# wzn0828/Adaptive

Hardware: AMD Instinct MI355X
Metric: captions/sec (greedy, max_len=20) at B=512; 1/2/4/8-GPU scaling (higher is better)
Workload: dtype fp32; 1 GPU; greedy decode (Encoder2Decoder.sampler) B=512/GPU, max_len=20; batch_per_gpu=512, global_batch=512, max_len=20, hidden=512, embed=256, vocab=10123, parallelism=dp1, batches_in_flight=1, feature_buffers=3, headline=one sampler() call after another on resident batches

## Files before the change

### adaptive_amd/csrc/aa_encoder.hip

```cpp
#include "aa_internal.hpp"

namespace aa {

__global__ __launch_bounds__(256) void k_avgpool(const float* __restrict__ feats, int64_t nch, float* __restrict__ a_g) {
  __shared__ float buf[4][64 * P];
  const int lane = threadIdx.x & 63, w = threadIdx.x >> 6;
  const int64_t ch0 = ((int64_t)blockIdx.x * 4 + w) * 64;
  const int nhere = ch0 < nch ? (int)(nch - ch0 < 64 ? nch - ch0 : 64) : 0;
  const int nf4 = nhere * P / 4;
  const float4* src = reinterpret_cast<const float4*>(feats + ch0 * P);
  float4* dst = reinterpret_cast<float4*>(buf[w]);
  for (int q = lane; q < nf4; q += 64) dst[q] = src[q];
  __syncthreads();
  if (lane < nhere) {
    const float* row = buf[w] + lane * P;
    float s = 0.f;
    for (int p = 0; p < P; ++p) s += row[p];
    a_g[ch0 + lane] = s / 49.0f;
  }
}

template <int BM>
struct ANCHW {
  const float* base;
  __device__ __forceinline__ void init(const float* F, int C, int m0, int M) {
    const int m = m0 + (int)(threadIdx.x % BM);
    const int mc = m < M ? m : M - 1;
    const int b = mc / P, p = mc - b * P;
    base = F + (int64_t)b * C * P + p;
  }
  __device__ __forceinline__ void map(int q, int& r, int& kq) const { r = q % BM; kq = q / BM; }
  __device__ __forceinline__ float4 load(int , int q, int k0) const {
    const float* s = base + (k0 + 4 * (q / BM)) * P;
    return make_float4(s[0], s[P], s[2 * P], s[3 * P]);
  }
};

__global__ __launch_bounds__(256) void k_enc_v(const float* __restrict__ feats, int B, int C, int H,
                                               const float* __restrict__ W, const float* __restrict__ bias,
                                               float* __restrict__ V) {
  constexpr int BM = 64, BN = 64;
  __shared__ __attribute__((aligned(16))) float lds[Tile<BM, BN>::LDS_FLOATS];
  const int M = B * P, MT = (M + BM - 1) / BM, NTn = H / BN;
  const int L = xcd_remap(blockIdx.x, MT * NTn);
  const int mt = L / NTn, nt = L % NTn;
  ANCHW<BM> al;
  al.init(feats, C, mt * BM, M);
  WRowMajor wl{W, C, nt * BN};
  floatx16 acc[1][1];
  gemm_mainloop<BM, BN>(al, wl, C / BK, lds, acc);
  const int lane = threadIdx.x & 63, wave = threadIdx.x >> 6, wm = wave >> 1, wn = wave & 1;
  const int col = nt * BN + wn * 32 + (lane & 31);
  const float bv = bias[col];
#pragma unroll
  for (int r = 0; r < 16; ++r) {
    const int row = mt * BM + wm * 32 + acc_row(r, lane);
    if (row < M) V[(int64_t)row * H + col] = reluf_(acc[0][0][r] + bv);
  }
}

constexpr int EV_BM = 128, EV_BN = 128, EV_BK = 32, EV_LD = 40;


__global__ __launch_bounds__(256, 2) void k_enc_v3(const float* __restrict__ feats, int B, int C, int H,
                                                   const bf16x8* __restrict__ W3, const float* __restrict__ bias,
                                                   float* __restrict__ V) {
  __shared__ __attribute__((aligned(16))) __bf16 As[2][3][EV_BM * EV_LD];
  const int M = B * P, MT = (M + EV_BM - 1) / EV_BM, NTn = H / EV_BN, KC = C / 16;
  const int L = xcd_remap(blockIdx.x, MT * NTn);
  const int mt = L / NTn, nt = L % NTn;
  const int t = threadIdx.x, lane = t & 63, wave = t >> 6;
  const int li = lane & 31, lh = lane >> 5;
  const int r = t & (EV_BM - 1), kh = t >> 7;
  int m = mt * EV_BM + r;
  m = m < M ? m : M - 1;
  const int bi = m / P, pi = m - bi * P;
  const float* arow = feats + (int64_t)bi * C * P + pi + (int64_t)(16 * kh) * P;
  const int nb0 = (nt * EV_BN + wave * 32) / 32;
  const bf16x8* wf0 = W3 + (size_t)nb0 * KC * 3 * 64 + lane;
  float ra[16];
  bf16x8 wa[2][3], wb[2][3];
  floatx16 acc[4];
#pragma unroll
  for (int a = 0; a < 4; ++a)
#pragma unroll
    for (int i = 0; i < 16; ++i) acc[a][i] = 0.f;

  auto gload_a = [&](int s) {
    const float* src = arow + (int64_t)(EV_BK * s) * P;
#pragma unroll
    for (int i = 0; i < 16; ++i) ra[i] = src[i * P];
  };
  auto gload_w = [&](int s, bf16x8 (&w)[2][3]) {
#pragma unroll
    for (int sub = 0; sub < 2; ++sub)
#pragma unroll
      for (int q = 0; q < 3; ++q) w[sub][q] = wf0[((size_t)(2 * s + sub) * 3 + q) * 64];
  };
  auto lstore_a = [&](int buf) {
    bf16x8 h[2], md[2], lo[2];
#pragma unroll
    for (int i = 0; i < 16; ++i) {
      __bf16 x0, x1, x2;
      split3(ra[i], x0, x1, x2);
      h[i >> 3][i & 7] = x0;
      md[i >> 3][i & 7] = x1;
      lo[i >> 3][i & 7] = x2;
    }
    const int o = r * EV_LD + 16 * kh;
#pragma unroll
    for (int j = 0; j < 2; ++j) {
      *reinterpret_cast<bf16x8*>(&As[buf][0][o + 8 * j]) = h[j];
      *reinterpret_cast<bf16x8*>(&As[buf][1][o + 8 * j]) = md[j];
      *reinterpret_cast<bf16x8*>(&As[buf][2][o + 8 * j]) = lo[j];
    }
  };
  auto compute = [&](int buf, const bf16x8 (&w)[2][3]) {
#pragma unroll
    for (int sub = 0; sub < 2; ++sub) {
#pragma unroll
      for (int a = 0; a < 4; ++a) {
        bf16x8 fa[3];
#pragma unroll
        for (int q = 0; q < 3; ++q)
          fa[q] = *reinterpret_cast<const bf16x8*>(&As[buf][q][(a * 32 + li) * EV_LD + 16 * sub + 8 * lh]);
        floatx16 x = acc[a];
        x = __builtin_amdgcn_mfma_f32_32x32x16_bf16(fa[2], w[sub][0], x, 0, 0, 0);
        x = __builtin_amdgcn_mfma_f32_32x32x16_bf16(fa[1], w[sub][1], x, 0, 0, 0);
        x = __builtin_amdgcn_mfma_f32_32x32x16_bf16(fa[0], w[sub][2], x, 0, 0, 0);
        x = __builtin_amdgcn_mfma_f32_32x32x16_bf16(fa[1], w[sub][0], x, 0, 0, 0);
        x = __builtin_amdgcn_mfma_f32_32x32x16_bf16(fa[0], w[sub][1], x, 0, 0, 0);
        x = __builtin_amdgcn_mfma_f32_32x32x16_bf16(fa[0], w[sub][0], x, 0, 0, 0);
        acc[a] = x;
      }
    }
  };

  const int ns = C / EV_BK;
  gload_a(0);
  gload_w(0, wa);
  lstore_a(0);
  gload_a(1);
  gload_w(1, wb);
  __syncthreads();
  for (int s = 0; s < ns; s += 2) {
    const int s2 = s + 2 < ns ? s + 2 : ns - 1, s3 = s + 3 < ns ? s + 3 : ns - 1;
    lstore_a(1);
    gload_a(s2);
    __builtin_amdgcn_sched_barrier(0);
    compute(0, wa);
    gload_w(s2, wa);
    __syncthreads();
    __builtin_amdgcn_sched_barrier(0);
    lstore_a(0);
    gload_a(s3);
    __builtin_amdgcn_sched_barrier(0);
    compute(1, wb);
    gload_w(s3, wb);
    __syncthreads();
    __builtin_amdgcn_sched_barrier(0);
  }
  const int col = nt * EV_BN + wave * 32 + li;
  const float bv = bias[col];
#pragma unroll
  for (int a = 0; a < 4; ++a)
#pragma unroll
    for (int i = 0; i < 16; ++i) {
      const int row = mt * EV_BM + a * 32 + acc_row(i, lane);
      if (row < M) V[(int64_t)row * H + col] = reluf_(acc[a][i] + bv);
    }
}

constexpr int E4_ROWS = 98, E4_RB = 7, E4_LD = 48;
constexpr int E4_SP = 52, E4_MAXC = 2048;
typedef float floatx4 __attribute__((ext_vector_type(4)));

constexpr int ENC4_NW = 16;

template <bool F>
struct BoolC {
  static constexpr bool value = F;
};

template <int NCB, int NW = 8>
__global__ __launch_bounds__(64 * NW) void k_enc_v4(const float* __restrict__ feats, int B, int C,
                                                const bf16x8* __restrict__ W4, const f16x8* __restrict__ W4h,
                                                const float* __restrict__ w4h_sc, const float* __restrict__ bias,
                                                float* __restrict__ V, float* __restrict__ a_g, int x3_only) {
  static_assert(NCB % 2 == 0, "columns are processed in pairs of 16-column blocks");
  constexpr int H = 16 * NCB * NW, NPAIR = NCB / 2, PL = E4_RB * 16 * E4_LD;
  constexpr int NT = 64 * NW;
  const bool stager = NW == 8 || threadIdx.x < 512;
  __shared__ __attribute__((aligned(16))) __bf16 As[2][3][PL];
  __shared__ __attribute__((aligned(16))) float Sg[2][2 * 32 * E4_SP];
  __shared__ __attribute__((aligned(16))) float Ag[2 * E4_MAXC];
  __shared__ int over_any;
  const int M = B * P, KC = C / 32;
  const int t = threadIdx.x, lane = t & 63, wave = t >> 6;
  const int m0 = blockIdx.x * E4_ROWS;
  const int sr = t < 4 * E4_ROWS ? t % E4_ROWS : E4_ROWS + (t & 7);
  const int kg = t < 4 * E4_ROWS ? t / E4_ROWS : (t >> 3) & 3;
  const bool stg = stager;
  int m = m0 + (t < 4 * E4_ROWS ? sr : 0);
  m = m < M ? m : M - 1;
  const int bi = m / P, pi = m - bi * P;
  const float* arow = feats + (int64_t)bi * C * P + pi + (int64_t)(8 * kg) * P;
  const int so = sr * E4_LD + 8 * kg;
  const int fo = (lane & 15) * E4_LD + 8 * (lane >> 4);
  floatx4 acc[E4_RB][NCB];

  auto kloop = [&](auto f16) -> bool {
    constexpr bool F16 = decltype(f16)::value;
    constexpr int NPL = F16 ? 2 : 3;
    const bf16x8* wsrc = (F16 ? reinterpret_cast<const bf16x8*>(W4h) : W4) + (size_t)(wave * NCB) * KC * NPL * 64 +
                         lane;
    float ra[8];
    bf16x8 wv[NCB][NPL];
    bool over = false;
#pragma unroll
    for (int rb = 0; rb < E4_RB; ++rb)
#pragma unroll
      for (int c = 0; c < NCB; ++c) acc[rb][c] = floatx4{0.f, 0.f, 0.f, 0.f};

    auto gload_a = [&](int s) {
      const float* src = arow + (int64_t)(32 * s) * P;
#pragma unroll
      for (int i = 0; i < 8; ++i) ra[i] = __builtin_nontemporal_load(src + i * P);
    };
    auto gload_w = [&](int s, int c) {
#pragma unroll
      for (int q = 0; q < NPL; ++q) wv[c][q] = wsrc[((size_t)c * KC * NPL + (size_t)s * NPL + q) * 64];
    };
    auto lstore_a = [&](int buf) {
      if constexpr (F16) {
        f16x8 x[2];
#pragma unroll
        for (int i = 0; i < 8; ++i) {
          _Float16 hi, lo;
          split2h(ra[i] * (float)(1 << ENC_F16_A_EXP), hi, lo);
          x[0][i] = hi; x[1][i] = lo;
          over |= !(__builtin_fabsf(ra[i]) < ENC_F16_A_MAX);
        }
#pragma unroll
        for (int q = 0; q < 2; ++q) *reinterpret_cast<bf16x8*>(&As[buf][q][so]) = __builtin_bit_cast(bf16x8, x[q]);
      } else {
        bf16x8 x[3];
#pragma unroll
        for (int i = 0; i < 8; ++i) {
          __bf16 x0, x1, x2;
          split3(ra[i], x0, x1, x2);
          x[0][i] = x0; x[1][i] = x1; x[2][i] = x2;
        }
#pragma unroll
        for (int q = 0; q < 3; ++q) *reinterpret_cast<bf16x8*>(&As[buf][q][so]) = x[q];
      }
      if (t < 4 * E4_ROWS) {
        const int img = sr >= P, pp = sr - img * P;
        float* g = &Sg[buf][(img * 32 + 8 * kg) * E4_SP + pp];
#pragma unroll
        for (int i = 0; i < 8; ++i) g[i * E4_SP] = ra[i];
      }
    };

    const int ns = KC;
    if (stg) gload_a(0);
#pragma unroll
    for (int c = 0; c < NCB; ++c) gload_w(0, c);
    if (stg) lstore_a(0);
    if (stg) gload_a(ns > 1 ? 1 : 0);
    __syncthreads();
    for (int s = 0; s < ns; ++s) {
      const int buf = s & 1, s1 = s + 1 < ns ? s + 1 : ns - 1, s2 = s + 2 < ns ? s + 2 : ns - 1;
      if (stg) {
        lstore_a(buf ^ 1);
        gload_a(s2);
      }
      __builtin_amdgcn_sched_barrier(0);
      const __bf16* Ab = &As[buf][0][fo];
#pragma unroll
      for (int cp = 0; cp < NPAIR; ++cp) {
#pragma unroll
        for (int rb = 0; rb < E4_RB; ++rb) {
          bf16x8 fa[NPL];
#pragma unroll
          for (int q = 0; q < NPL; ++q) fa[q] = *reinterpret_cast<const bf16x8*>(Ab + q * PL + rb * 16 * E4_LD);
          const int c0 = 2 * cp, c1 = c0 + 1;
          floatx4 x = acc[rb][c0], y = acc[rb][c1];
          if constexpr (F16) {
            const f16x8 ah = __builtin_bit_cast(f16x8, fa[0]), al = __builtin_bit_cast(f16x8, fa[1]);
            const f16x8 w0h = __builtin_bit_cast(f16x8, wv[c0][0]), w0l = __builtin_bit_cast(f16x8, wv[c0][1]);
            const f16x8 w1h = __builtin_bit_cast(f16x8, wv[c1][0]), w1l = __builtin_bit_cast(f16x8, wv[c1][1]);
            x = __builtin_amdgcn_mfma_f32_16x16x32_f16(al, w0h, x, 0, 0, 0);
            y = __builtin_amdgcn_mfma_f32_16x16x32_f16(al, w1h, y, 0, 0, 0);
            x = __builtin_amdgcn_mfma_f32_16x16x32_f16(ah, w0l, x, 0, 0, 0);
            y = __builtin_amdgcn_mfma_f32_16x16x32_f16(ah, w1l, y, 0, 0, 0);
            x = __builtin_amdgcn_mfma_f32_16x16x32_f16(ah, w0h, x, 0, 0, 0);
            y = __builtin_amdgcn_mfma_f32_16x16x32_f16(ah, w1h, y, 0, 0, 0);
          } else {
            x = __builtin_amdgcn_mfma_f32_16x16x32_bf16(fa[2], wv[c0][0], x, 0, 0, 0);
            y = __builtin_amdgcn_mfma_f32_16x16x32_bf16(fa[2], wv[c1][0], y, 0, 0, 0);
            x = __builtin_amdgcn_mfma_f32_16x16x32_bf16(fa[1], wv[c0][1], x, 0, 0, 0);
            y = __builtin_amdgcn_mfma_f32_16x16x32_bf16(fa[1], wv[c1][1], y, 0, 0, 0);
            x = __builtin_amdgcn_mfma_f32_16x16x32_bf16(fa[0], wv[c0][2], x, 0, 0, 0);
            y = __builtin_amdgcn_mfma_f32_16x16x32_bf16(fa[0], wv[c1][2], y, 0, 0, 0);
            x = __builtin_amdgcn_mfma_f32_16x16x32_bf16(fa[1], wv[c0][0], x, 0, 0, 0);
            y = __builtin_amdgcn_mfma_f32_16x16x32_bf16(fa[1], wv[c1][0], y, 0, 0, 0);
            x = __builtin_amdgcn_mfma_f32_16x16x32_bf16(fa[0], wv[c0][1], x, 0, 0, 0);
            y = __builtin_amdgcn_mfma_f32_16x16x32_bf16(fa[0], wv[c1][1], y, 0, 0, 0);
            x = __builtin_amdgcn_mfma_f32_16x16x32_bf16(fa[0], wv[c0][0], x, 0, 0, 0);
            y = __builtin_amdgcn_mfma_f32_16x16x32_bf16(fa[0], wv[c1][0], y, 0, 0, 0);
          }
          acc[rb][c0] = x;
          acc[rb][c1] = y;
        }
        gload_w(s1, 2 * cp);
        gload_w(s1, 2 * cp + 1);
        asm volatile("" ::: "memory");
      }
      if (wave == (s & 7)) {
        const float* g = &Sg[buf][lane * E4_SP];
        float sum = 0.f;
#pragma unroll 4
        for (int pp = 0; pp < 48; pp += 4) {
          const float4 v = *reinterpret_cast<const float4*>(g + pp);
          sum += v.x; sum += v.y; sum += v.z; sum += v.w;
        }
        sum += g[48];
        Ag[(lane >> 5) * C + 32 * s + (lane & 31)] = sum / 49.0f;
      }
      __syncthreads();
      __builtin_amdgcn_sched_barrier(0);
    }
    return over;
  };

  bool x3 = x3_only != 0;
  float unscale = 1.0f;
  if (!x3) {
    if (t == 0) over_any = 0;
    if (kloop(BoolC<true>{})) over_any = 1;
    __syncthreads();
    x3 = over_any != 0;
    unscale = w4h_sc[0];
  }
  if (x3) {
    kloop(BoolC<false>{});
    unscale = 1.0f;
  }
  for (int i = t; i < 2 * C; i += NT) {
    const int img = 2 * blockIdx.x + (i >= C);
    if (img < B) a_g[(int64_t)img * C + (i - (i >= C ? C : 0))] = Ag[i];
  }
  float* Vs = reinterpret_cast<float*>(&As[0][0][0]);
  constexpr int VSP = H + 4;
  static_assert(16 * VSP * 4 <= sizeof(As), "V staging must fit in the A stages");
  float bvs[NCB];
#pragma unroll
  for (int c = 0; c < NCB; ++c) bvs[c] = bias[(wave * NCB + c) * 16 + (lane & 15)];
#pragma unroll
  for (int rb = 0; rb < E4_RB; ++rb) {
    __syncthreads();
#pragma unroll
    for (int c = 0; c < NCB; ++c) {
      const int col = (wave * NCB + c) * 16 + (lane & 15);
#pragma unroll
      for (int i = 0; i < 4; ++i)
        Vs[(4 * (lane >> 4) + i) * VSP + col] = reluf_(acc[rb][c][i] * unscale + bvs[c]);
    }
    __syncthreads();
    constexpr int F4 = 16 * H / 4;
#pragma unroll
    for (int q = t; q < F4; q += NT) {
      const int r = q / (H / 4), c4 = q % (H / 4), tr = rb * 16 + r, row = m0 + tr;
      if (tr < E4_ROWS && row < M)
        *reinterpret_cast<float4*>(V + (int64_t)row * H + 4 * c4) = *reinterpret_cast<const float4*>(Vs + r * VSP + 4 * c4);
    }
  }
}

__global__ __launch_bounds__(256) void k_enc_heads(const float* __restrict__ a_g, int B, int C, int E, int H, int NHp,
                                                   const float* __restrict__ W, const float* __restrict__ bias,
                                                   float* __restrict__ v_g, float* __restrict__ h0, float* __restrict__ c0) {
  constexpr int BM = 64, BN = 64;
  __shared__ __attribute__((aligned(16))) float lds[Tile<BM, BN>::LDS_FLOATS];
  const int MT = (B + BM - 1) / BM, NTn = NHp / BN;
  const int L = xcd_remap(blockIdx.x, MT * NTn);
  const int nt = L / MT, mt = L % MT;
  ARowMajor al{a_g, C, mt * BM, B};
  WRowMajor wl{W, C, nt * BN};
  floatx16 acc[1][1];
  gemm_mainloop<BM, BN>(al, wl, C / BK, lds, acc);
  const int lane = threadIdx.x & 63, wave = threadIdx.x >> 6, wm = wave >> 1, wn = wave & 1;
  const int col = nt * BN + wn * 32 + (lane & 31);
  if (col >= E + 2 * H) return;
  const float bv = bias[col];
#pragma unroll
  for (int r = 0; r < 16; ++r) {
    const int row = mt * BM + wm * 32 + acc_row(r, lane);
    if (row >= B) continue;
    const float x = acc[0][0][r] + bv;
    if (col < E) v_g[(int64_t)row * E + col] = reluf_(x);
    else if (col < E + H) h0[(int64_t)row * H + (col - E)] = tanhf(x);
    else c0[(int64_t)row * H + (col - E - H)] = tanhf(x);
  }
}

enum { MODE_HEADS = 0, MODE_PLAIN = 1 };
template <int NB, int NWV, int MODE>
__global__ __launch_bounds__(64 * NWV) void k_gemm3(const float* __restrict__ A, int M, int K, int N,
                                                    const bf16x8* __restrict__ W4, const float* __restrict__ bias,
                                                    float* __restrict__ out0, int ldo, float* __restrict__ h0,
                                                    float* __restrict__ c0, int E, int H,
                                                    bf16x8* __restrict__ hsp = nullptr, int64_t* __restrict__ tok0 = nullptr,
                                                    int tok_n = 0, uint64_t* __restrict__ keys = nullptr, int key_n = 0) {
  constexpr int BN = 16 * NB, TP = BN + 4;
  if (MODE == MODE_HEADS && tok0) {
    const int i0 = blockIdx.x * blockDim.x + threadIdx.x, stride = gridDim.x * blockDim.x;
    for (int i = i0; i < tok_n; i += stride) tok0[i] = 1;
    for (int i = i0; i < key_n; i += stride) __hip_atomic_store(keys + i, 0ull, __ATOMIC_RELAXED, __HIP_MEMORY_SCOPE_AGENT);
  }
  __shared__ __attribute__((aligned(16))) float Pt[NWV][32 * TP];
  const int KC = K / 32, NTn = (N + BN - 1) / BN;
  const int mt = blockIdx.x / NTn, nt = blockIdx.x % NTn;
  const int t = threadIdx.x, lane = t & 63, wave = t >> 6;
  const int m0 = mt * 32;
  const float* arow[2];
#pragma unroll
  for (int rb = 0; rb < 2; ++rb) {
    int m = m0 + 16 * rb + (lane & 15);
    m = m < M ? m : M - 1;
    arow[rb] = A + (int64_t)m * K + 8 * (lane >> 4);
  }
  const bf16x8* wsrc = W4 + (size_t)(nt * NB) * KC * 3 * 64 + lane;
  floatx4 acc[2][NB];
#pragma unroll
  for (int rb = 0; rb < 2; ++rb)
#pragma unroll
    for (int c = 0; c < NB; ++c) acc[rb][c] = floatx4{0.f, 0.f, 0.f, 0.f};
  const int per = KC / NWV, kc0 = wave * per;
  float4 av[2][2][2];
  bf16x8 wv[2][NB][3];
  auto load = [&](int slot, int kc) {
#pragma unroll
    for (int rb = 0; rb < 2; ++rb) {
      av[slot][rb][0] = *reinterpret_cast<const float4*>(arow[rb] + 32 * kc);
      av[slot][rb][1] = *reinterpret_cast<const float4*>(arow[rb] + 32 * kc + 4);
    }
#pragma unroll
    for (int c = 0; c < NB; ++c)
#pragma unroll
      for (int q = 0; q < 3; ++q) wv[slot][c][q] = wsrc[((size_t)c * KC * 3 + (size_t)kc * 3 + q) * 64];
  };
  auto step = [&](int slot) {
#pragma unroll
    for (int rb = 0; rb < 2; ++rb) {
      bf16x8 fa[3];
#pragma unroll
      for (int i = 0; i < 8; ++i) {
        __bf16 x0, x1, x2;
        split3(f4c(av[slot][rb][i >> 2], i & 3), x0, x1, x2);
        fa[0][i] = x0; fa[1][i] = x1; fa[2][i] = x2;
      }
#pragma unroll
      for (int c = 0; c < NB; ++c) {
        floatx4 x = acc[rb][c];
        x = __builtin_amdgcn_mfma_f32_16x16x32_bf16(fa[2], wv[slot][c][0], x, 0, 0, 0);
        x = __builtin_amdgcn_mfma_f32_16x16x32_bf16(fa[1], wv[slot][c][1], x, 0, 0, 0);
        x = __builtin_amdgcn_mfma_f32_16x16x32_bf16(fa[0], wv[slot][c][2], x, 0, 0, 0);
        x = __builtin_amdgcn_mfma_f32_16x16x32_bf16(fa[1], wv[slot][c][0], x, 0, 0, 0);
        x = __builtin_amdgcn_mfma_f32_16x16x32_bf16(fa[0], wv[slot][c][1], x, 0, 0, 0);
        x = __builtin_amdgcn_mfma_f32_16x16x32_bf16(fa[0], wv[slot][c][0], x, 0, 0, 0);
        acc[rb][c] = x;
      }
    }
  };
  const int last = kc0 + per - 1;
  load(0, kc0);
  load(1, kc0 + 1 < last ? kc0 + 1 : last);
  for (int kc = kc0; kc < kc0 + per; kc += 2) {
    step(0);
    load(0, kc + 2 < last ? kc + 2 : last);
    step(1);
    load(1, kc + 3 < last ? kc + 3 : last);
  }
#pragma unroll
  for (int rb = 0; rb < 2; ++rb)
#pragma unroll
    for (int c = 0; c < NB; ++c)
#pragma unroll
      for (int i = 0; i < 4; ++i) Pt[wave][(16 * rb + 4 * (lane >> 4) + i) * TP + 16 * c + (lane & 15)] = acc[rb][c][i];
  __syncthreads();
  for (int e = t; e < 32 * BN; e += 64 * NWV) {
    const int r = e / BN, cl = e - r * BN, row = m0 + r, col = nt * BN + cl;
    if (row >= M || col >= N) continue;
    const int o = r * TP + cl;
    float ps[NWV];
#pragma unroll
    for (int w = 0; w < NWV; ++w) ps[w] = Pt[w][o];
#pragma unroll
    for (int st = 1; st < NWV; st *= 2)
#pragma unroll
      for (int w = 0; w + st < NWV; w += 2 * st) ps[w] += ps[w + st];
    if (MODE == MODE_PLAIN) {
      out0[(int64_t)row * ldo + col] = bias ? ps[0] + bias[col] : ps[0];
    } else {
      const float x = ps[0] + bias[col];
      if (col < E) out0[(int64_t)row * E + col] = reluf_(x);
      else if (col < E + H) {
        const float hv = tanhf(x);
        const int k = col - E;
        h0[(int64_t)row * H + k] = hv;
        if (hsp) {
          __bf16 x0, x1, x2;
          split3(hv, x0, x1, x2);
          __bf16* o = reinterpret_cast<__bf16*>(hsp + ((size_t)((row >> 5) * (H / 16) + (k >> 4)) * 3) * 64 +
                                                (row & 31) + 32 * ((k >> 3) & 1)) + (k & 7);
          o[0] = x0;
          o[64 * 8] = x1;
          o[128 * 8] = x2;
        }
      } else {
        c0[(int64_t)row * H + (col - E - H)] = tanhf(x);
      }
    }
  }
}

__global__ __launch_bounds__(256) void k_gemm_bias(const float* __restrict__ A, int lda, int M, const float* __restrict__ W,
                                                   int ldw, int N, int K, const float* __restrict__ bias,
                                                   float* __restrict__ Cm, int64_t ldc) {
  constexpr int BM = 64, BN = 64;
  __shared__ __attribute__((aligned(16))) float lds[Tile<BM, BN>::LDS_FLOATS];
  const int MT = (M + BM - 1) / BM, NTn = N / BN;
  const int L = xcd_remap(blockIdx.x, MT * NTn);
  const int nt = L / MT, mt = L % MT;
  ARowMajor al{A, lda, mt * BM, M};
  WRowMajor wl{W, ldw, nt * BN};
  floatx16 acc[1][1];
  gemm_mainloop<BM, BN>(al, wl, K / BK, lds, acc);
  const int lane = threadIdx.x & 63, wave = threadIdx.x >> 6, wm = wave >> 1, wn = wave & 1;
  const int col = nt * BN + wn * 32 + (lane & 31);
  const float bv = bias ? bias[col] : 0.f;
#pragma unroll
  for (int r = 0; r < 16; ++r) {
    const int row = mt * BM + wm * 32 + acc_row(r, lane);
    if (row < M) Cm[(int64_t)row * ldc + col] = bias ? acc[0][0][r] + bv : acc[0][0][r];
  }
}

__global__ void k_decode_init(int64_t* __restrict__ tok, int B, int64_t v, uint64_t* __restrict__ keys, int n) {
  const int i0 = blockIdx.x * blockDim.x + threadIdx.x, stride = gridDim.x * blockDim.x;
  for (int i = i0; i < B; i += stride) tok[i] = v;
  if (keys)
    for (int i = i0; i < n; i += stride) __hip_atomic_store(keys + i, 0ull, __ATOMIC_RELAXED, __HIP_MEMORY_SCOPE_AGENT);
}

__global__ void k_pack_lstm(const float* __restrict__ w_ih, const float* __restrict__ w_hh, const float* __restrict__ b_ih,
                            const float* __restrict__ b_hh, const float* __restrict__ w_x, int E, int H,
                            float* __restrict__ whh, float* __restrict__ wemb, float* __restrict__ wvg, float* __restrict__ bias5) {
  const int r = blockIdx.x;
  const int KX = 2 * E;
  if (r < 4 * H) {
    const int tile = r / 64, g = (r % 64) / 16, un = r % 16;
    const int src = g * H + tile * 16 + un;
    for (int k = threadIdx.x; k < E; k += blockDim.x) {
      wemb[(int64_t)r * E + k] = w_ih[(int64_t)src * KX + k];
      wvg[(int64_t)r * E + k] = w_ih[(int64_t)src * KX + E + k];
    }
    for (int k = threadIdx.x; k < H; k += blockDim.x) whh[(int64_t)r * H + k] = w_hh[(int64_t)src * H + k];
    if (threadIdx.x == 0) bias5[r] = b_ih[src] + b_hh[src];
  } else if (w_x) {
    const int j = r - 4 * H;
    for (int k = threadIdx.x; k < E; k += blockDim.x) {
      wemb[(int64_t)r * E + k] = w_x[(int64_t)j * KX + k];
      wvg[(int64_t)r * E + k] = w_x[(int64_t)j * KX + E + k];
    }
    if (threadIdx.x == 0) bias5[r] = 0.f;
  }
}

__global__ void k_pack_w3(const float* __restrict__ w, int C, bf16x8* __restrict__ out) {
  const int KC = C / 16, nb = blockIdx.x / KC, kc = blockIdx.x % KC, l = threadIdx.x;
  const float* src = w + (int64_t)(32 * nb + (l & 31)) * C + 16 * kc + 8 * (l >> 5);
  bf16x8 h, m, lo;
#pragma unroll
  for (int j = 0; j < 8; ++j) {
    __bf16 a, b, c;
    split3(src[j], a, b, c);
    h[j] = a; m[j] = b; lo[j] = c;
  }
  bf16x8* o = out + ((size_t)blockIdx.x * 3) * 64 + l;
  o[0] = h;
  o[64] = m;
  o[128] = lo;
}

__global__ void k_pack_w4(const float* __restrict__ w, int C, bf16x8* __restrict__ out) {
  const int KC = C / 32, nb = blockIdx.x / KC, kc = blockIdx.x % KC, l = threadIdx.x;
  const float* src = w + (int64_t)(16 * nb + (l & 15)) * C + 32 * kc + 8 * (l >> 4);
  bf16x8 h, m, lo;
#pragma unroll
  for (int j = 0; j < 8; ++j) {
    __bf16 a, b, c;
    split3(src[j], a, b, c);
    h[j] = a; m[j] = b; lo[j] = c;
  }
  bf16x8* o = out + ((size_t)blockIdx.x * 3) * 64 + l;
  o[0] = h;
  o[64] = m;
  o[128] = lo;
}

__global__ __launch_bounds__(1024) void k_w4h_scale(const float* __restrict__ w, size_t n, float* __restrict__ sc) {
  __shared__ uint32_t part[16];
  uint32_t mx = 0;
  for (size_t i = threadIdx.x; i < n; i += 1024) {
    const uint32_t u = __float_as_uint(w[i]) & 0x7FFFFFFFu;
    mx = u > mx ? u : mx;
  }
#pragma unroll
  for (int o = 32; o > 0; o >>= 1) {
    const uint32_t x = (uint32_t)__shfl_xor((int)mx, o, 64);
    mx = x > mx ? x : mx;
  }
  if ((threadIdx.x & 63) == 0) part[threadIdx.x >> 6] = mx;
  __syncthreads();
  if (threadIdx.x == 0) {
    for (int i = 1; i < 16; ++i) mx = part[i] > mx ? part[i] : mx;
    const int be = (int)(mx >> 23);
    int e = be == 0 || be == 255 ? 0 : ENC_F16_W_TOP - (be - 127);
    e = e > ENC_F16_W_ECLAMP ? ENC_F16_W_ECLAMP : e < -ENC_F16_W_ECLAMP ? -ENC_F16_W_ECLAMP : e;
    sc[0] = ldexpf(1.0f, -(e + ENC_F16_A_EXP));
    sc[1] = (float)e;
  }
}
__global__ void k_pack_w4h(const float* __restrict__ w, int C, const float* __restrict__ sc, f16x8* __restrict__ out) {
  const int KC = C / 32, nb = blockIdx.x / KC, kc = blockIdx.x % KC, l = threadIdx.x;
  const float* src = w + (int64_t)(16 * nb + (l & 15)) * C + 32 * kc + 8 * (l >> 4);
  const float scale = ldexpf(1.0f, (int)sc[1]);
  f16x8 h, lo;
#pragma unroll
  for (int j = 0; j < 8; ++j) {
    _Float16 a, b;
    split2h(src[j] * scale, a, b);
    h[j] = a; lo[j] = b;
  }
  f16x8* o = out + ((size_t)blockIdx.x * 2) * 64 + l;
  o[0] = h;
  o[64] = lo;
}

__global__ void k_pack_wgs(const float* __restrict__ wg, const float* __restrict__ ws, int H, float* __restrict__ out) {
  const int tile = blockIdx.x;
  for (int i = threadIdx.x; i < (ws ? 2 : 1) * P * 16; i += blockDim.x) {
    const int j = i / 16, u = i % 16;
    const float* src = j < P ? wg + (int64_t)j * H : ws + (int64_t)(j - P) * H;
    out[(int64_t)tile * 2 * P * 16 + i] = src[tile * 16 + u];
  }
}

__global__ void k_pack_mlp(const float* __restrict__ w, int V, int H, int Vp, uint16_t* __restrict__ wb,
                           float* __restrict__ wn) {
  const int n = blockIdx.x, lane = threadIdx.x;
  float s = 0.f, sd = 0.f;
  for (int k = lane; k < H; k += 64) {
    const float x = n < V ? w[(int64_t)n * H + k] : 0.f;
    const uint16_t xb = f2bf(x);
    wb[frag_off(n, k, H)] = xb;
    const float d = x - __uint_as_float((uint32_t)xb << 16);
    s = __builtin_fmaf(x, x, s);
    sd = __builtin_fmaf(d, d, sd);
  }
  s = wave_sum(s);
  sd = wave_sum(sd);
  if (lane == 0) {
    wn[n] = sqrtf(s) * 1.0001f;
    wn[Vp + n] = sqrtf(sd) * 1.0001f;
  }
}

__global__ void k_pack_gs(const float* __restrict__ wn, const float* __restrict__ b, int Vp, float4* __restrict__ gs) {
  const int g = blockIdx.x, l = threadIdx.x;
  const int n = g * VS_TILE + (l & (VS_TILE - 1));
  const float mw = wave_max(wn[n]), mb = wave_max(fabsf(b[n])), md = wave_max(wn[Vp + n]);
  if (l == 0) gs[g] = make_float4(mw, mb, md, 0.f);
}

}

using namespace aa;

namespace aa {

void gemm_bias(const float* A, int lda, int M, const float* W, int ldw, int N, int K, const float* bias, float* C,
                      int64_t ldc, hipStream_t s) {
  const int MT = (M + 63) / 64, NTn = N / 64;
  hipLaunchKernelGGL(k_gemm_bias, dim3(MT * NTn), dim3(256), 0, s, A, lda, M, W, ldw, N, K, bias, C, ldc);
}
void avgpool_launch(const float* feats, int64_t nch, float* a_g, hipStream_t s) {
  hipLaunchKernelGGL(k_avgpool, dim3((unsigned)((nch + 255) / 256)), dim3(256), 0, s, feats, nch, a_g);
}
void enc_v_launch(const float* feats, int B, int C, int H, const float* w, const float* b, float* V, hipStream_t s) {
  const int M = B * P, MT = (M + 63) / 64, NTn = H / 64;
  hipLaunchKernelGGL(k_enc_v, dim3(MT * NTn), dim3(256), 0, s, feats, B, C, H, w, b, V);
}

}

int aa_pack_weights(const aa_model* m, const aa_ref_weights* w, aa_stream_t stream) {
  Layout L;
  int rc = check_model(m, &L);
  if (rc) return rc;
  if (!w) return AA_ERR_NULL;
  const float* req[] = {w->enc_affine_a_w, w->enc_affine_a_b, w->enc_affine_b_w, w->enc_affine_b_b,
                        w->enc_affine_h0_w, w->enc_affine_h0_b, w->enc_affine_c0_w, w->enc_affine_c0_b,
                        w->embed_w, w->lstm_w_ih, w->lstm_w_hh, w->lstm_b_ih, w->lstm_b_hh,
                        w->att_affine_v_w, w->att_affine_g_w, w->att_affine_h_w, w->mlp_w, w->mlp_b};
  for (const float* p : req)
    if (!p) return AA_ERR_NULL;
  const bool baseline = !w->sent_affine_x_w && !w->att_affine_s_w;
  if (!baseline && (!w->sent_affine_x_w || !w->att_affine_s_w)) return AA_ERR_NULL;
  if (!al16(w->embed_w)) return AA_ERR_ALIGN;
  hipStream_t s = (hipStream_t)stream;
  float* base = static_cast<float*>(m->packed);
  const int E = L.E, H = L.H, V = L.V, C = L.C;
  AA_TRY(hipMemsetAsync(base, 0, L.total_floats * sizeof(float), s));
  auto cp = [&](const float* src, size_t off, size_t n) {
    return hipMemcpyAsync(base + off, src, n * sizeof(float), hipMemcpyDeviceToDevice, s);
  };
  AA_TRY(cp(w->enc_affine_a_w, L.enc_a_w, (size_t)H * C));
  AA_TRY(cp(w->enc_affine_a_b, L.enc_a_b, H));
  AA_TRY(cp(w->enc_affine_b_w, L.heads_w, (size_t)E * C));
  AA_TRY(cp(w->enc_affine_h0_w, L.heads_w + (size_t)E * C, (size_t)H * C));
  AA_TRY(cp(w->enc_affine_c0_w, L.heads_w + (size_t)(E + H) * C, (size_t)H * C));
  AA_TRY(cp(w->enc_affine_b_b, L.heads_b, E));
  AA_TRY(cp(w->enc_affine_h0_b, L.heads_b + E, H));
  AA_TRY(cp(w->enc_affine_c0_b, L.heads_b + E + H, H));
  AA_TRY(cp(w->att_affine_v_w, L.wv, (size_t)P * H));
  AA_TRY(cp(w->att_affine_g_w, L.wg, (size_t)P * H));
  if (!baseline) AA_TRY(cp(w->att_affine_s_w, L.ws, (size_t)P * H));
  AA_TRY(cp(w->att_affine_h_w, L.wh, P));
  AA_TRY(cp(w->mlp_w, L.mlp_w, (size_t)V * H));
  AA_TRY(cp(w->mlp_b, L.mlp_b, V));
  hipLaunchKernelGGL(k_pack_lstm, dim3(L.N5), dim3(256), 0, s, w->lstm_w_ih, w->lstm_w_hh, w->lstm_b_ih, w->lstm_b_hh,
                     w->sent_affine_x_w, E, H, base + L.whh, base + L.wemb, base + L.wvg, base + L.bias5);
  gemm_bias(w->embed_w, E, V, base + L.wemb, E, L.N5, E, nullptr, base + L.table, L.N5, s);
  hipLaunchKernelGGL(k_pack_mlp, dim3(L.Vp), dim3(64), 0, s, base + L.mlp_w, V, H, L.Vp,
                     reinterpret_cast<uint16_t*>(base + L.mlp_wb), base + L.mlp_wn);
  hipLaunchKernelGGL(k_pack_gs, dim3(L.Vp / VS_TILE), dim3(64), 0, s, base + L.mlp_wn, base + L.mlp_b, L.Vp,
                     reinterpret_cast<float4*>(base + L.mlp_gs));
  hipLaunchKernelGGL(k_pack_wgs, dim3(H / 16), dim3(256), 0, s, w->att_affine_g_w, w->att_affine_s_w, H, base + L.wgs);
  hipLaunchKernelGGL(k_pack_w3, dim3((H / 32) * (C / 16)), dim3(64), 0, s, w->enc_affine_a_w, C,
                     reinterpret_cast<bf16x8*>(base + L.enc_w3));
  hipLaunchKernelGGL(k_pack_w3, dim3((4 * H / 32) * (H / 16)), dim3(64), 0, s, base + L.whh, H,
                     reinterpret_cast<bf16x8*>(base + L.whh3));
  hipLaunchKernelGGL(k_pack_w3, dim3((L.Vp / 32) * (H / 16)), dim3(64), 0, s, base + L.mlp_w, H,
                     reinterpret_cast<bf16x8*>(base + L.mlp_w3));
  hipLaunchKernelGGL(k_pack_w4, dim3((H / 16) * (C / 32)), dim3(64), 0, s, w->enc_affine_a_w, C,
                     reinterpret_cast<bf16x8*>(base + L.enc_w4));
  hipLaunchKernelGGL(k_w4h_scale, dim3(1), dim3(1024), 0, s, w->enc_affine_a_w, (size_t)H * C, base + L.enc_w4h_sc);
  hipLaunchKernelGGL(k_pack_w4h, dim3((H / 16) * (C / 32)), dim3(64), 0, s, w->enc_affine_a_w, C,
                     (const float*)(base + L.enc_w4h_sc), reinterpret_cast<f16x8*>(base + L.enc_w4h));
  hipLaunchKernelGGL(k_pack_w4, dim3((L.NHp / 16) * (C / 32)), dim3(64), 0, s, base + L.heads_w, C,
                     reinterpret_cast<bf16x8*>(base + L.heads_w4));
  if (E % 32 == 0)
    hipLaunchKernelGGL(k_pack_w4, dim3((L.N5 / 16) * (E / 32)), dim3(64), 0, s, base + L.wvg, E,
                       reinterpret_cast<bf16x8*>(base + L.wvg4));
  if (H % 32 == 0)
    hipLaunchKernelGGL(k_pack_w4, dim3((PP / 16) * (H / 32)), dim3(64), 0, s, base + L.wv, H,
                       reinterpret_cast<bf16x8*>(base + L.wv4));
  return launch_status();
}

static bool enc_v4(const Layout& L, int32_t flags) {
  return !(flags & AA_DECODE_FP32_ENCODER) && (L.H == 512 || L.H == 256) && L.C <= E4_MAXC;
}
static bool gemm3_ok(int32_t flags, int K) {
  return !(flags & AA_DECODE_FP32_ENCODER) && K % 256 == 0;
}
int aa::encoder_launch(const Layout& L, const MP& p, const float* feats, int B, float* a_g, float* V, float* v_g,
                   float* h0, float* c0, float* VWv, float* xg, aa_event_t* ev, int32_t flags, hipStream_t s,
                   hipStream_t aux, bf16x8* hsp0, const DecodeInit* init) {
  const int C = L.C, H = L.H, E = L.E;
  const int64_t nch = (int64_t)B * C;
  hipEvent_t fork = nullptr, join = nullptr, heads_done = nullptr;
  hipStream_t sa = s;
  if (aux && aux != s) {
    AA_TRY(hipEventCreateWithFlags(&fork, hipEventDisableTiming));
    AA_TRY(hipEventCreateWithFlags(&join, hipEventDisableTiming));
    if (hsp0) AA_TRY(hipEventCreateWithFlags(&heads_done, hipEventDisableTiming));
    AA_TRY(hipEventRecord(fork, s));
    AA_TRY(hipStreamWaitEvent(aux, fork, 0));
    sa = aux;
  }
  const bool heads_split = hsp0 && !(flags & AA_DECODE_FP32_ENCODER || C % 256) && (E + 2 * H) % 80 == 0 && C % 512 == 0;
  const bool init_in_heads = init && sa == s && !(flags & AA_DECODE_FP32_ENCODER || C % 256) &&
                             (E + 2 * H) % 80 == 0 && C % 512 == 0;
  if (init && !init_in_heads) {
    const int nblk = init->n / 256 + 1;
    hipLaunchKernelGGL(k_decode_init, dim3(nblk < 1024 ? nblk : 1024), dim3(256), 0, sa, init->tok0, init->B,
                       (int64_t)1, init->keys, init->n);
  }
  auto heads_xg = [&](hipStream_t st) {
    const int NH = E + 2 * H;
    if (flags & AA_DECODE_FP32_ENCODER || C % 256) {
      const int MT = (B + 63) / 64, NTn = L.NHp / 64;
      AA_TLAUNCH(ev, 4, k_enc_heads, dim3(MT * NTn), dim3(256), 0, st, a_g, B, C, E, H, L.NHp, p.heads_w, p.heads_b,
                 v_g, h0, c0);
    } else if (NH % 80 == 0 && C % 512 == 0) {
      AA_TLAUNCH(ev, 4, (k_gemm3<5, 8, MODE_HEADS>), dim3(((B + 31) / 32) * (NH / 80)), dim3(512), 0, st,
                 (const float*)a_g, B, C, NH, (const bf16x8*)p.heads_w4, (const float*)p.heads_b, v_g, 0, h0, c0, E, H,
                 heads_split ? hsp0 : (bf16x8*)nullptr, init_in_heads ? init->tok0 : (int64_t*)nullptr,
                 init_in_heads ? init->B : 0, init_in_heads ? init->keys : (uint64_t*)nullptr,
                 init_in_heads ? init->n : 0);
    } else {
      AA_TLAUNCH(ev, 4, (k_gemm3<4, 4, MODE_HEADS>), dim3(((B + 31) / 32) * ((NH + 63) / 64)), dim3(256), 0, st,
                 (const float*)a_g, B, C, NH, (const bf16x8*)p.heads_w4, (const float*)p.heads_b, v_g, 0, h0, c0, E, H,
                 (bf16x8*)nullptr, (int64_t*)nullptr, 0, (uint64_t*)nullptr, 0);
    }
    if (heads_done) (void)hipEventRecord(heads_done, st);
    if (xg && gemm3_ok(flags, E) && L.N5 % 80 == 0) {
      AA_TLAUNCH(ev, 8, (k_gemm3<5, 4, MODE_PLAIN>), dim3(((B + 31) / 32) * (L.N5 / 80)), dim3(256), 0, st,
                 (const float*)v_g, B, E, L.N5, (const bf16x8*)p.wvg4, (const float*)p.bias5, xg, L.N5, (float*)nullptr,
                 (float*)nullptr, 0, 0, (bf16x8*)nullptr, (int64_t*)nullptr, 0, (uint64_t*)nullptr, 0);
    } else if (xg) {
      rec(ev, 8, st);
      gemm_bias(v_g, E, B, p.wvg, E, L.N5, E, p.bias5, xg, L.N5, st);
      rec(ev, 9, st);
    }
  };
  const bool v4 = enc_v4(L, flags);
  if (v4) {
    const int nwg = (B * P + E4_ROWS - 1) / E4_ROWS;
    const int x3_only = (flags & AA_DECODE_ENC_BF16X3) != 0;
    if (H == 512)
      AA_TLAUNCH(ev, 2, (k_enc_v4<32 / ENC4_NW, ENC4_NW>), dim3(nwg), dim3(64 * ENC4_NW), 0, s, feats, B, C,
                 (const bf16x8*)p.enc_w4, (const f16x8*)p.enc_w4h, (const float*)p.enc_w4h_sc, (const float*)p.enc_a_b,
                 V, a_g, x3_only);
    else
      AA_TLAUNCH(ev, 2, k_enc_v4<2>, dim3(nwg), dim3(512), 0, s, feats, B, C, (const bf16x8*)p.enc_w4,
                 (const f16x8*)p.enc_w4h, (const float*)p.enc_w4h_sc, (const float*)p.enc_a_b, V, a_g, x3_only);
    if (sa != s) {
      hipEvent_t agr = nullptr;
      AA_TRY(hipEventCreateWithFlags(&agr, hipEventDisableTiming));
      AA_TRY(hipEventRecord(agr, s));
      AA_TRY(hipStreamWaitEvent(sa, agr, 0));
      AA_TRY(hipEventDestroy(agr));
    }
    heads_xg(sa);
  } else {
    AA_TLAUNCH(ev, 0, k_avgpool, dim3((unsigned)((nch + 255) / 256)), dim3(256), 0, sa, feats, nch, a_g);
    heads_xg(sa);
    if (flags & AA_DECODE_FP32_ENCODER) {
      const int M = B * P, MT = (M + 63) / 64, NTn = H / 64;
      AA_TLAUNCH(ev, 2, k_enc_v, dim3(MT * NTn), dim3(256), 0, s, feats, B, C, H, (const float*)p.enc_a_w,
                 (const float*)p.enc_a_b, V);
    } else {
      const int M = B * P, MT = (M + EV_BM - 1) / EV_BM, NTn = H / EV_BN;
      AA_TLAUNCH(ev, 2, k_enc_v3, dim3(MT * NTn), dim3(256), 0, s, feats, B, C, H, (const bf16x8*)p.enc_w3,
                 (const float*)p.enc_a_b, V);
    }
  }
  if (VWv && gemm3_ok(flags, H)) {
    AA_TLAUNCH(ev, 6, (k_gemm3<4, 4, MODE_PLAIN>), dim3((B * P + 31) / 32), dim3(256), 0, s, (const float*)V, B * P, H,
               PP, (const bf16x8*)p.wv4, (const float*)nullptr, VWv, PP, (float*)nullptr, (float*)nullptr, 0, 0,
               (bf16x8*)nullptr, (int64_t*)nullptr, 0, (uint64_t*)nullptr, 0);
  } else if (VWv) {
    rec(ev, 6, s);
    gemm_bias(V, H, B * P, p.wv, H, PP, H, nullptr, VWv, PP, s);
    rec(ev, 7, s);
  }
  if (hsp0 && !heads_split) {
    if (heads_done) AA_TRY(hipStreamWaitEvent(s, heads_done, 0));
    split_rows_launch(h0, B, H, hsp0, s);
  }
  if (heads_done) AA_TRY(hipEventDestroy(heads_done));
  if (join) {
    AA_TRY(hipEventRecord(join, sa));
    AA_TRY(hipStreamWaitEvent(s, join, 0));
    AA_TRY(hipEventDestroy(join));
    AA_TRY(hipEventDestroy(fork));
  }
  return launch_status();
}

int aa_encoder_tail(const aa_model* m, const float* feats, int32_t B, float* a_g, float* V, float* v_g, float* h0,
                    float* c0, float* VWv, int32_t flags, aa_stream_t stream) {
  Layout L;
  int rc = check_model(m, &L);
  if (rc) return rc;
  if (B < 0) return AA_ERR_SHAPE;
  if (B == 0) return AA_OK;
  if (!feats || !a_g || !V || !v_g || !h0 || !c0) return AA_ERR_NULL;
  if (!al16(feats) || !al16(a_g) || !al16(V) || !al16(VWv) || !al16(v_g)) return AA_ERR_ALIGN;
  return encoder_launch(L, resolve(m, L), feats, B, a_g, V, v_g, h0, c0, VWv, nullptr, nullptr, flags,
                        (hipStream_t)stream);
}
```

Measured before the change: 511,400 captions/s.

## Deepen encoder A-staging ring to four stages and halve block barriers in f16 path

Turns the encoder GEMM's double-buffered LDS staging of the activation tiles into a ring of four stages on the two-plane f16 path, with prefetch distance two, and syncs the block only every other k-step. The stager/non-stager split becomes a wave-uniform compile-time role, so the pipeline loop is specialised without per-thread predicates. The goal is fewer __syncthreads stalls and more latency hiding for global feature loads. In exchange it uses more LDS (a larger As plus four Sg buffers), which may reduce occupancy, and with syncs every other step a wave can run up to two stages ahead. Correctness depends on that distance staying within the ring.

```diff
diff --git a/adaptive_amd/csrc/aa_encoder.hip b/adaptive_amd/csrc/aa_encoder.hip
--- a/adaptive_amd/csrc/aa_encoder.hip
+++ b/adaptive_amd/csrc/aa_encoder.hip
@@ -190,17 +190,17 @@
   static_assert(NCB % 2 == 0, "columns are processed in pairs of 16-column blocks");
   constexpr int H = 16 * NCB * NW, NPAIR = NCB / 2, PL = E4_RB * 16 * E4_LD;
   constexpr int NT = 64 * NW;
-  const bool stager = NW == 8 || threadIdx.x < 512;
-  __shared__ __attribute__((aligned(16))) __bf16 As[2][3][PL];
-  __shared__ __attribute__((aligned(16))) float Sg[2][2 * 32 * E4_SP];
+  __shared__ __attribute__((aligned(16))) __bf16 As[8 * PL];
+  __shared__ __attribute__((aligned(16))) float Sg[4][2 * 32 * E4_SP];
   __shared__ __attribute__((aligned(16))) float Ag[2 * E4_MAXC];
   __shared__ int over_any;
+  static_assert(sizeof(As) + sizeof(Sg) + sizeof(Ag) + sizeof(int) <= 160 * 1024, "LDS of one CU");
   const int M = B * P, KC = C / 32;
   const int t = threadIdx.x, lane = t & 63, wave = t >> 6;
   const int m0 = blockIdx.x * E4_ROWS;
   const int sr = t < 4 * E4_ROWS ? t % E4_ROWS : E4_ROWS + (t & 7);
   const int kg = t < 4 * E4_ROWS ? t / E4_ROWS : (t >> 3) & 3;
-  const bool stg = stager;
+  const bool stg_wave = NW == 8 || __builtin_amdgcn_readfirstlane(threadIdx.x >> 6) < 8;
   int m = m0 + (t < 4 * E4_ROWS ? sr : 0);
   m = m < M ? m : M - 1;
   const int bi = m / P, pi = m - bi * P;
@@ -211,7 +211,7 @@
 
   auto kloop = [&](auto f16) -> bool {
     constexpr bool F16 = decltype(f16)::value;
-    constexpr int NPL = F16 ? 2 : 3;
+    constexpr int NPL = F16 ? 2 : 3, RING = F16 ? 4 : 2, D = RING / 2;
     const bf16x8* wsrc = (F16 ? reinterpret_cast<const bf16x8*>(W4h) : W4) + (size_t)(wave * NCB) * KC * NPL * 64 +
                          lane;
     float ra[8];
@@ -223,7 +223,7 @@
       for (int c = 0; c < NCB; ++c) acc[rb][c] = floatx4{0.f, 0.f, 0.f, 0.f};
 
     auto gload_a = [&](int s) {
-      const float* src = arow + (int64_t)(32 * s) * P;
+      const float* src = arow + (int64_t)(32 * (s < KC ? s : KC - 1)) * P;
 #pragma unroll
       for (int i = 0; i < 8; ++i) ra[i] = __builtin_nontemporal_load(src + i * P);
     };
@@ -242,7 +242,7 @@
           over |= !(__builtin_fabsf(ra[i]) < ENC_F16_A_MAX);
         }
 #pragma unroll
-        for (int q = 0; q < 2; ++q) *reinterpret_cast<bf16x8*>(&As[buf][q][so]) = __builtin_bit_cast(bf16x8, x[q]);
+        for (int q = 0; q < 2; ++q) *reinterpret_cast<bf16x8*>(&As[(buf * NPL + q) * PL + so]) = __builtin_bit_cast(bf16x8, x[q]);
       } else {
         bf16x8 x[3];
 #pragma unroll
@@ -252,7 +252,7 @@
           x[0][i] = x0; x[1][i] = x1; x[2][i] = x2;
         }
 #pragma unroll
-        for (int q = 0; q < 3; ++q) *reinterpret_cast<bf16x8*>(&As[buf][q][so]) = x[q];
+        for (int q = 0; q < 3; ++q) *reinterpret_cast<bf16x8*>(&As[(buf * NPL + q) * PL + so]) = x[q];
       }
       if (t < 4 * E4_ROWS) {
         const int img = sr >= P, pp = sr - img * P;
@@ -263,73 +263,87 @@
     };
 
     const int ns = KC;
-    if (stg) gload_a(0);
-#pragma unroll
-    for (int c = 0; c < NCB; ++c) gload_w(0, c);
-    if (stg) lstore_a(0);
-    if (stg) gload_a(ns > 1 ? 1 : 0);
-    __syncthreads();
-    for (int s = 0; s < ns; ++s) {
-      const int buf = s & 1, s1 = s + 1 < ns ? s + 1 : ns - 1, s2 = s + 2 < ns ? s + 2 : ns - 1;
-      if (stg) {
-        lstore_a(buf ^ 1);
-        gload_a(s2);
-      }
-      __builtin_amdgcn_sched_barrier(0);
-      const __bf16* Ab = &As[buf][0][fo];
-#pragma unroll
-      for (int cp = 0; cp < NPAIR; ++cp) {
-#pragma unroll
-        for (int rb = 0; rb < E4_RB; ++rb) {
-          bf16x8 fa[NPL];
-#pragma unroll
-          for (int q = 0; q < NPL; ++q) fa[q] = *reinterpret_cast<const bf16x8*>(Ab + q * PL + rb * 16 * E4_LD);
-          const int c0 = 2 * cp, c1 = c0 + 1;
-          floatx4 x = acc[rb][c0], y = acc[rb][c1];
-          if constexpr (F16) {
-            const f16x8 ah = __builtin_bit_cast(f16x8, fa[0]), al = __builtin_bit_cast(f16x8, fa[1]);
-            const f16x8 w0h = __builtin_bit_cast(f16x8, wv[c0][0]), w0l = __builtin_bit_cast(f16x8, wv[c0][1]);
-            const f16x8 w1h = __builtin_bit_cast(f16x8, wv[c1][0]), w1l = __builtin_bit_cast(f16x8, wv[c1][1]);
-            x = __builtin_amdgcn_mfma_f32_16x16x32_f16(al, w0h, x, 0, 0, 0);
-            y = __builtin_amdgcn_mfma_f32_16x16x32_f16(al, w1h, y, 0, 0, 0);
-            x = __builtin_amdgcn_mfma_f32_16x16x32_f16(ah, w0l, x, 0, 0, 0);
-            y = __builtin_amdgcn_mfma_f32_16x16x32_f16(ah, w1l, y, 0, 0, 0);
-            x = __builtin_amdgcn_mfma_f32_16x16x32_f16(ah, w0h, x, 0, 0, 0);
-            y = __builtin_amdgcn_mfma_f32_16x16x32_f16(ah, w1h, y, 0, 0, 0);
-          } else {
-            x = __builtin_amdgcn_mfma_f32_16x16x32_bf16(fa[2], wv[c0][0], x, 0, 0, 0);
-            y = __builtin_amdgcn_mfma_f32_16x16x32_bf16(fa[2], wv[c1][0], y, 0, 0, 0);
-            x = __builtin_amdgcn_mfma_f32_16x16x32_bf16(fa[1], wv[c0][1], x, 0, 0, 0);
-            y = __builtin_amdgcn_mfma_f32_16x16x32_bf16(fa[1], wv[c1][1], y, 0, 0, 0);
-            x = __builtin_amdgcn_mfma_f32_16x16x32_bf16(fa[0], wv[c0][2], x, 0, 0, 0);
-            y = __builtin_amdgcn_mfma_f32_16x16x32_bf16(fa[0], wv[c1][2], y, 0, 0, 0);
-            x = __builtin_amdgcn_mfma_f32_16x16x32_bf16(fa[1], wv[c0][0], x, 0, 0, 0);
-            y = __builtin_amdgcn_mfma_f32_16x16x32_bf16(fa[1], wv[c1][0], y, 0, 0, 0);
-            x = __builtin_amdgcn_mfma_f32_16x16x32_bf16(fa[0], wv[c0][1], x, 0, 0, 0);
-            y = __builtin_amdgcn_mfma_f32_16x16x32_bf16(fa[0], wv[c1][1], y, 0, 0, 0);
-            x = __builtin_amdgcn_mfma_f32_16x16x32_bf16(fa[0], wv[c0][0], x, 0, 0, 0);
-            y = __builtin_amdgcn_mfma_f32_16x16x32_bf16(fa[0], wv[c1][0], y, 0, 0, 0);
-          }
-          acc[rb][c0] = x;
-          acc[rb][c1] = y;
+    auto stages = [&](auto role) {
+      constexpr bool STG = decltype(role)::value;
+      if constexpr (STG) gload_a(0);
+#pragma unroll
+      for (int c = 0; c < NCB; ++c) gload_w(0, c);
+      if constexpr (STG) {
+#pragma unroll
+        for (int d = 0; d < D; ++d) {
+          lstore_a(d);
+          gload_a(d + 1);
         }
-        gload_w(s1, 2 * cp);
-        gload_w(s1, 2 * cp + 1);
-        asm volatile("" ::: "memory");
-      }
-      if (wave == (s & 7)) {
-        const float* g = &Sg[buf][lane * E4_SP];
-        float sum = 0.f;
-#pragma unroll 4
-        for (int pp = 0; pp < 48; pp += 4) {
-          const float4 v = *reinterpret_cast<const float4*>(g + pp);
-          sum += v.x; sum += v.y; sum += v.z; sum += v.w;
-        }
-        sum += g[48];
-        Ag[(lane >> 5) * C + 32 * s + (lane & 31)] = sum / 49.0f;
       }
       __syncthreads();
-      __builtin_amdgcn_sched_barrier(0);
+      for (int s = 0; s < ns; ++s) {
+        const int buf = s & (RING - 1), s1 = s + 1 < ns ? s + 1 : ns - 1;
+        if constexpr (STG) {
+          lstore_a((s + D) & (RING - 1));
+          gload_a(s + D + 1);
+        }
+        __builtin_amdgcn_sched_barrier(0);
+        const __bf16* Ab = &As[buf * NPL * PL + fo];
+#pragma unroll
+        for (int cp = 0; cp < NPAIR; ++cp) {
+#pragma unroll
+          for (int rb = 0; rb < E4_RB; ++rb) {
+            bf16x8 fa[NPL];
+#pragma unroll
+            for (int q = 0; q < NPL; ++q) fa[q] = *reinterpret_cast<const bf16x8*>(Ab + q * PL + rb * 16 * E4_LD);
+            const int c0 = 2 * cp, c1 = c0 + 1;
+            floatx4 x = acc[rb][c0], y = acc[rb][c1];
+            if constexpr (F16) {
+              const f16x8 ah = __builtin_bit_cast(f16x8, fa[0]), al = __builtin_bit_cast(f16x8, fa[1]);
+              const f16x8 w0h = __builtin_bit_cast(f16x8, wv[c0][0]), w0l = __builtin_bit_cast(f16x8, wv[c0][1]);
+              const f16x8 w1h = __builtin_bit_cast(f16x8, wv[c1][0]), w1l = __builtin_bit_cast(f16x8, wv[c1][1]);
+              x = __builtin_amdgcn_mfma_f32_16x16x32_f16(al, w0h, x, 0, 0, 0);
+              y = __builtin_amdgcn_mfma_f32_16x16x32_f16(al, w1h, y, 0, 0, 0);
+              x = __builtin_amdgcn_mfma_f32_16x16x32_f16(ah, w0l, x, 0, 0, 0);
+              y = __builtin_amdgcn_mfma_f32_16x16x32_f16(ah, w1l, y, 0, 0, 0);
+              x = __builtin_amdgcn_mfma_f32_16x16x32_f16(ah, w0h, x, 0, 0, 0);
+              y = __builtin_amdgcn_mfma_f32_16x16x32_f16(ah, w1h, y, 0, 0, 0);
+            } else {
+              x = __builtin_amdgcn_mfma_f32_16x16x32_bf16(fa[2], wv[c0][0], x, 0, 0, 0);
+              y = __builtin_amdgcn_mfma_f32_16x16x32_bf16(fa[2], wv[c1][0], y, 0, 0, 0);
+              x = __builtin_amdgcn_mfma_f32_16x16x32_bf16(fa[1], wv[c0][1], x, 0, 0, 0);
+              y = __builtin_amdgcn_mfma_f32_16x16x32_bf16(fa[1], wv[c1][1], y, 0, 0, 0);
+              x = __builtin_amdgcn_mfma_f32_16x16x32_bf16(fa[0], wv[c0][2], x, 0, 0, 0);
+              y = __builtin_amdgcn_mfma_f32_16x16x32_bf16(fa[0], wv[c1][2], y, 0, 0, 0);
+              x = __builtin_amdgcn_mfma_f32_16x16x32_bf16(fa[1], wv[c0][0], x, 0, 0, 0);
+              y = __builtin_amdgcn_mfma_f32_16x16x32_bf16(fa[1], wv[c1][0], y, 0, 0, 0);
+              x = __builtin_amdgcn_mfma_f32_16x16x32_bf16(fa[0], wv[c0][1], x, 0, 0, 0);
+              y = __builtin_amdgcn_mfma_f32_16x16x32_bf16(fa[0], wv[c1][1], y, 0, 0, 0);
+              x = __builtin_amdgcn_mfma_f32_16x16x32_bf16(fa[0], wv[c0][0], x, 0, 0, 0);
+              y = __builtin_amdgcn_mfma_f32_16x16x32_bf16(fa[0], wv[c1][0], y, 0, 0, 0);
+            }
+            acc[rb][c0] = x;
+            acc[rb][c1] = y;
+          }
+          gload_w(s1, 2 * cp);
+          gload_w(s1, 2 * cp + 1);
+          asm volatile("" ::: "memory");
+        }
+        if (STG && wave == (s & 7)) {
+          const float* g = &Sg[buf][lane * E4_SP];
+          float sum = 0.f;
+#pragma unroll 4
+          for (int pp = 0; pp < 48; pp += 4) {
+            const float4 v = *reinterpret_cast<const float4*>(g + pp);
+            sum += v.x; sum += v.y; sum += v.z; sum += v.w;
+          }
+          sum += g[48];
+          Ag[(lane >> 5) * C + 32 * s + (lane & 31)] = sum / 49.0f;
+        }
+        if (D == 1 || (s & 1) || s == ns - 1) __syncthreads();
+        __builtin_amdgcn_sched_barrier(0);
+      }
+    };
+    if constexpr (NW == 8) {
+      stages(BoolC<true>{});
+    } else {
+      if (stg_wave) stages(BoolC<true>{});
+      else stages(BoolC<false>{});
     }
     return over;
   };
@@ -351,7 +365,7 @@
     const int img = 2 * blockIdx.x + (i >= C);
     if (img < B) a_g[(int64_t)img * C + (i - (i >= C ? C : 0))] = Ag[i];
   }
-  float* Vs = reinterpret_cast<float*>(&As[0][0][0]);
+  float* Vs = reinterpret_cast<float*>(&As[0]);
   constexpr int VSP = H + 4;
   static_assert(16 * VSP * 4 <= sizeof(As), "V staging must fit in the A stages");
   float bvs[NCB];
```

After: 515,400 captions/s (median of 6 runs). No clear change (+0.8%).
